# maxwellsh/DIGDriver

Measured on AMD Instinct MI355X. Metric: genomic elements tested/sec (whole node), whole-genome x 37 cohorts, higher is better.
Workload: dtype f64

## Files before the change

digdriver_amd/_lib.py:

```python
import ctypes
import os
import sys

import numpy as np

_HERE = os.path.dirname(os.path.abspath(__file__))
LIB_PATH = os.environ.get("DIG_HIP_LIB") or os.path.join(_HERE, "lib", "libdig_hip.so")

DIG_F32, DIG_F64, DIG_I16, DIG_BF16 = 0, 1, 2, 3
DIG_PIPE_CONTEXTS, DIG_PIPE_DOT, DIG_PIPE_STATISTICS, DIG_PIPE_WORKLIST_CLEAN, DIG_PIPE_COMPACT_L, DIG_PIPE_RECORDS = 1, 2, 4, 8, 16, 32
DIG_REC_DOUBLES, DIG_REC_MU, DIG_REC_SIGMA, DIG_REC_ROBS_FLAG = 10, 7, 8, 9
DIG_CNV_SCAN_CHUNK = 2048
GENE_CLASSES = ("SYN", "MIS", "NONS", "SPL", "TRUNC", "NONSYN")
GS_PLANES = tuple("EXP_" + c for c in GENE_CLASSES) + tuple("PVAL_%s_BURDEN" % c for c in GENE_CLASSES) + \
    tuple("PVAL_%s_BURDEN_SAMPLE" % c for c in GENE_CLASSES) + ("THETA_INDEL", "EXP_INDEL", "PVAL_INDEL_BURDEN", "PVAL_MUT_BURDEN")
SEL_PLANES = ("T_SYN", "MRFOLD") + tuple("EXP_%s_ML" % c for c in GENE_CLASSES) + \
    tuple("PVAL_%s_BURDEN_DNDS" % c for c in GENE_CLASSES) + tuple("PVAL_%s_SEL_NB" % c for c in ("SYN", "MIS", "TRUNC", "NONSYN")) + \
    tuple("PVAL_%s_SEL_PG" % c for c in ("SYN", "MIS", "NONS", "NONSYN")) + tuple("SEL_" + c for c in GENE_CLASSES) + \
    tuple("PVAL_%s_SEL" % c for c in GENE_CLASSES)
ES_PLANES = ("EXP_SNV", "PVAL_SNV_BURDEN", "PVAL_SAMPLE_BURDEN", "THETA_INDEL", "EXP_INDEL",
             "PVAL_INDEL_BURDEN", "PVAL_MUT_BURDEN")


class DigHipError(RuntimeError):
    pass


_lib = None
TORCH_FREE = False
_loaded_without_torch = False


def _need_torch():
# ... 11 lines not shown
    "dig_nb_exact_host": [_vp, _vp, _vp, _vp, _i64, _int],
    "dig_nb_greater": [_vp, _vp, _vp, _vp, _i64, _vp],
    "dig_nb_greater_host": [_vp, _vp, _vp, _vp, _i64, _int],
    "dig_nb_midp_twosided": [_vp, _vp, _vp, _vp, _i64, _vp],
    "dig_nb_midp_twosided_host": [_vp, _vp, _vp, _vp, _i64, _int],
    "dig_fisher": [_vp, _vp, _vp, _i64, _vp],
    "dig_fisher_host": [_vp, _vp, _vp, _i64, _int],
    "dig_normal_params_to_gamma": [_vp, _vp, _vp, _vp, _i64, _vp],
    "dig_normal_params_to_gamma_host": [_vp, _vp, _vp, _vp, _i64, _int],
    "dig_element_stats": [_vp, _vp, _vp, _vp, _vp, _vp, _int, _vp, _vp, _vp, _vp, _vp, _vp, _i64, _i64, _vp, _i64, _vp],
    "dig_element_stats_host": [_vp, _vp, _vp, _vp, _vp, _vp, _int, _vp, _vp, _vp, _vp, _vp, _vp, _i64, _i64, _int],
    "dig_accumulate_elements": [_vp] * 8 + [_int] + [_vp] * 11 + [_i64, _i64, _i64, _vp, _i64, _vp],
    "dig_accumulate_elements_host": [_vp] * 8 + [_int] + [_vp] * 11 + [_i64, _i64, _i64, _int],
    "dig_scale_suffstats": [_vp, _vp, _i64, _i64, _vp, _vp, _i64, _vp],
    "dig_scale_suffstats_host": [_vp, _vp, _i64, _i64, _vp, _int],
    "dig_scale_factors": [_vp, _int, _i64, _vp, _vp, _vp],
    "dig_scale_suffstats_chunked": [_vp, _vp, _i64, _vp, _int, _vp, _vp, _i64, _vp],
    "dig_scale_factors_chunked": [_vp, _int, _vp, _int, _i64, _vp, _vp, _vp, _vp],
    "dig_scale_factors_local": [_vp, _vp, _i64, _i64, _vp, _vp, _vp, _vp, _vp, _vp, _i64, _vp],
    "dig_element_pipeline": [_vp] * 25 + [_i64, _i64, _i64, _vp, _int, _vp, _i64, _vp],
    "dig_bin_records_pack": [_vp, _vp, _vp, _vp, _i64, _i64, _vp, _i64, _vp],
    "dig_element_records_unpack": [_vp, _i64, _i64, _vp, _vp, _vp, _vp, _vp, _int, _vp],
    "dig_element_pipeline_prepare": [_vp, _i64, _i64, _vp, _i64, _vp, _vp],
    "dig_element_pipeline_host": [_vp] * 25 + [_i64, _i64, _i64, _int],
    "dig_gene_stats": [_vp, _vp, _vp, _vp, _vp, _int, _vp, _int, _vp, _vp, _vp, _vp, _int, _vp, _i64, _i64, _vp],
    "dig_gene_stats_host": [_vp, _vp, _vp, _vp, _vp, _int, _vp, _int, _vp, _vp, _vp, _vp, _int, _vp, _i64, _i64, _int],
    "dig_gene_selection": [_vp, _vp, _vp, _int, _vp, _vp, _i64, _i64, _vp],
    "dig_gene_selection_host": [_vp, _vp, _vp, _int, _vp, _vp, _i64, _i64, _int],
    "dig_gene_row_keys": [_vp] * 5 + [_i64] * 4 + [_vp, _vp, _vp],
    "dig_gene_row_keys_host": [_vp] * 5 + [_i64] * 4 + [_vp, _vp, _int],
    "dig_gene_counts": [_vp, _i64, _vp, _i64, ctypes.c_double, ctypes.c_double, _i64, _i64, _i64] + [_vp] * 7,
    "dig_gene_counts_host": [_vp, _i64, _vp, _i64, ctypes.c_double, ctypes.c_double, _i64, _i64, _i64] + [_vp] * 5 + [_int],
    "dig_panel_row_keys": [_vp] * 7 + [_i64] * 5 + [_vp, _vp, _vp],
    "dig_panel_row_keys_host": [_vp] * 7 + [_i64] * 5 + [_vp, _vp, _int],
    "dig_panel_counts": [_vp, _i64, _vp, _vp] + [_i64] * 4 + [_vp] * 4,
    "dig_panel_counts_host": [_vp, _i64, _vp, _vp] + [_i64] * 4 + [_vp] * 3 + [_int],
    "dig_window_pair_keys": [_vp, _vp, _i64, _vp, _i64, _vp, _vp, _vp] + [_i64] * 4 + [_vp, _vp],
    "dig_window_pair_keys_host": [_vp, _vp, _i64, _vp, _i64, _vp, _vp, _vp] + [_i64] * 4 + [_vp, _int],
    "dig_window_sample_hits": [_vp] + [_i64] * 4 + [_vp, _vp],
    "dig_window_sample_hits_host": [_vp] + [_i64] * 4 + [_vp, _int],
    "dig_window_objectives": [_vp, _i64, _vp, _vp] + [_i64] * 4 + [_vp, _vp, _vp],
    "dig_window_objectives_host": [_vp, _i64, _vp, _vp] + [_i64] * 4 + [_vp, _int],
    "dig_cnv_segment_deltas": [_vp, _vp, _vp, _i64, _i64, _i64] + [_vp] * 6 + [_i64, _i64, _vp, _vp],
    "dig_cnv_segment_deltas_host": [_vp, _vp, _vp, _i64, _i64, _i64] + [_vp] * 6 + [_i64, _i64, _vp, _int],
    "dig_cnv_window_means": [_vp, _i64, _i64, _i64, _vp, _vp, _vp],
    "dig_cnv_window_means_host": [_vp, _i64, _i64, _i64, _vp, _int],
# ... 248 lines not shown
```

digdriver_amd/csrc/dig_accumulate.hip:

```cpp
#include <algorithm>
#include <type_traits>
#include <vector>

#include "dig_common.hpp"
#include "dig_math.hpp"

namespace dig {

constexpr int kAccLdsBudget = 160 * 1024 - 1024;

struct AccArgs {
    const double *bin_mu, *bin_std;
    const int32_t* bin_y;
    const uint8_t* bin_flag;
    const int32_t* bin_ctx;
    const int64_t* ov_ptr;
    const int32_t* ov_idx;
    const int32_t* L;
    const uint8_t* strand_minus;
    const int32_t* gene_length;
    const double* d_pr;
    double *MU, *SIGMA;
    int32_t *R_OBS, *FLAG;
    double* P;
// ... 494 lines not shown
            }
        }
        tile = tile_next;
    }
}

constexpr int kCtxWaves = 12;
constexpr int kCtxSteps = 16;

__global__ __launch_bounds__(256) void compact_L_kernel(const int32_t* __restrict__ L, int64_t n64, int32_t* __restrict__ Lc,
                                                        int* __restrict__ mismatch)
{
    const int64_t stride = (int64_t)gridDim.x * 256;
    int bad = 0;
    for (int64_t g = (int64_t)blockIdx.x * 256 + threadIdx.x; g < n64; g += stride) {
        const int32_t* p = L + 3 * g;
        const int a = p[0], b = p[1], c = p[2];
        Lc[g] = a;
        bad |= (a != b) | (a != c);
    }
    if (__any(bad) && (threadIdx.x & 63) == 0) atomicOr(mismatch, 1);
}

template <int NT, int NQ>
__global__ __launch_bounds__(kCtxWaves * 64) __attribute__((amdgpu_waves_per_eu(3, 3), amdgpu_num_vgpr(80))) void acc_dot_ctx_kernel(
    const int32_t* __restrict__ bin_ctx, const int64_t* __restrict__ ov_ptr, const int32_t* __restrict__ ov_idx,
    const uint8_t* __restrict__ strand_minus, const int32_t* __restrict__ Lc, const double* __restrict__ d_pr,
    const int32_t* __restrict__ gene_length, double* __restrict__ P, int32_t* __restrict__ R_SIZE,
    int32_t* __restrict__ ELT_SIZE, double* __restrict__ P_INDEL, int64_t E, int C, int c0, int write_sizes,
    unsigned* __restrict__ zero_dwords, int n_zero)
{
    constexpr int SL = NT + (NQ > 0 ? 1 : 0);
    constexpr int NTA = NT > 0 ? NT : 1, NQA = NQ > 0 ? NQ : 1;
    __shared__ double tab[kCtxSteps * SL * 64];

    if (zero_dwords && blockIdx.x == 0 && (int)threadIdx.x < n_zero) zero_dwords[threadIdx.x] = 0u;
    if (threadIdx.x < kChunkCohorts) g_cohort_bad[threadIdx.x] = 0u;
    __syncthreads();

    const int lane = threadIdx.x & 63, wave = __builtin_amdgcn_readfirstlane((int)(threadIdx.x >> 6));
    const int i = lane & 15, kq = lane >> 4;
    const int toff = 4 * kq + (lane & 3);
    const int64_t n_tiles = (E + 15) >> 4;
    const int nx = (gridDim.x & 7u) == 0u ? 8 : 1;
    const int xcd = blockIdx.x % nx, slot_b = blockIdx.x / nx, nslots = gridDim.x / nx;
    const int64_t per_x = (n_tiles + nx - 1) / nx;
    const int64_t t_begin = (int64_t)xcd * per_x;
    const int64_t t_end = t_begin + per_x < n_tiles ? t_begin + per_x : n_tiles;
    const int64_t stride = (int64_t)nslots * kCtxWaves;
    int64_t tile = t_begin + (int64_t)wave * nslots + slot_b;

    const int4* ctx4 = reinterpret_cast<const int4*>(bin_ctx);
    const int4* L4 = reinterpret_cast<const int4*>(Lc);
    const int64_t nnz = ov_ptr[E];
    const int32_t* oi_base = nnz > 0 ? ov_idx : reinterpret_cast<const int32_t*>(ov_ptr);
    const int64_t oi_last = nnz > 0 ? nnz - 1 : 0;

    struct Bounds { int64_t q0; int cm; };
    struct Idx { int i0, i1; };
    struct Rows { int4 a[4], b[4], l[4]; };
    auto first_row = [&](int64_t tile_) { return min(tile_, n_tiles - 1) * 16; };
    auto row_off = [&](int64_t row0) { return (unsigned)min(i, (int)min(E - 1 - row0, (int64_t)15)); };
    auto load_bounds = [&](int64_t tile_) {
        Bounds r;
        const int64_t row0 = first_row(tile_);
        const unsigned ro = row_off(row0);
        const int64_t* op = ov_ptr + row0;
        r.q0 = op[ro];
        const int cnt = (int)(op[ro + 1] - r.q0);
        r.cm = max(cnt, 0) | ((strand_minus + row0)[ro] ? (int)0x80000000u : 0);
        return r;
    };
    auto load_idx = [&](const Bounds& b) {
        Idx x;
        x.i0 = oi_base[min(b.q0, oi_last)];
        x.i1 = oi_base[min(b.q0 + 1, oi_last)];
        return x;
    };
    auto load_rows = [&](int64_t tile_, const Bounds& b, const Idx& x) {
        Rows r;
        const int kk = b.cm < 0 ? 3 - kq : kq;
        const int4* r0 = ctx4 + (int64_t)x.i0 * 16 + kk;
        const int4* r1 = ctx4 + (int64_t)x.i1 * 16 + kk;
        const int64_t row0 = first_row(tile_);
        const int4* rl = L4 + row0 * 16;
        const unsigned lo = row_off(row0) * 16u + (unsigned)kq;
#pragma unroll
        for (int t = 0; t < 4; ++t) r.a[t] = r0[4 * t];
#pragma unroll
        for (int t = 0; t < 4; ++t) r.b[t] = r1[4 * t];
#pragma unroll
        for (int t = 0; t < 4; ++t) r.l[t] = rl[lo + 4u * t];
        return r;
    };

    Bounds b_c = load_bounds(tile), b_n = load_bounds(tile + stride);
    Idx x_c = load_idx(b_c);

    {
        constexpr int kTotal = kCtxSteps * SL * 64;
        constexpr int kPer = (kTotal + kCtxWaves * 64 - 1) / (kCtxWaves * 64);
        double d0[kPer], d1[kPer], d2[kPer];
#pragma unroll
        for (int j = 0; j < kPer; ++j) {
            const int idx = threadIdx.x + j * kCtxWaves * 64;
            const int lane_ = idx & 63, slot = (idx >> 6) % SL, step = idx / (SL * 64);
            const bool tail = NQ > 0 && slot == NT;
            const int kappa = 16 * (step >> 2) + 4 * (tail ? (lane_ >> 2) & 3 : lane_ >> 4) + (step & 3);
            const int c = c0 + slot * 16 + (tail ? 4 * (lane_ >> 4) + (lane_ & 3) : lane_ & 15);
            d0[j] = d1[j] = d2[j] = 0.0;
            if (idx < kTotal && c < C && (!tail || (lane_ >> 4) < NQ)) {
                const double* d = d_pr + (int64_t)c * 192 + 3 * kappa;
                d0[j] = d[0];
// ... 2 lines not shown
                if (!(d0[j] > 0.0 && d1[j] > 0.0 && d2[j] > 0.0)) atomicOr(&g_cohort_bad[c - c0], 1u);
            }
        }
#pragma unroll
        for (int j = 0; j < kPer; ++j) {
            const int idx = threadIdx.x + j * kCtxWaves * 64;
            if (idx < kTotal) tab[idx] = (d0[j] + d1[j]) + d2[j];
        }
    }
    Rows r_c = load_rows(tile, b_c, x_c);
    __syncthreads();
    if (tile >= t_end) return;

    while (tile < t_end) {
        int opaque_zero;
        asm volatile("s_mov_b32 %0, 0" : "=s"(opaque_zero));
        const double* tabw = tab + opaque_zero;
        const int64_t e0 = tile * 16;
        const Bounds b_nn = load_bounds(tile + 2 * stride);
        const Idx x_n = load_idx(b_n);
        const int cnt = b_c.cm & 0x7fffffff;
        const bool minus = b_c.cm < 0;
        int rcv[4][4], lv[4][4];
        {
            const int m0 = cnt > 0 ? -1 : 0, m1 = cnt > 1 ? -1 : 0;
#pragma unroll
            for (int t = 0; t < 4; ++t) {
                rcv[t][0] = (r_c.a[t].x & m0) + (r_c.b[t].x & m1);
                rcv[t][1] = (r_c.a[t].y & m0) + (r_c.b[t].y & m1);
                rcv[t][2] = (r_c.a[t].z & m0) + (r_c.b[t].z & m1);
                rcv[t][3] = (r_c.a[t].w & m0) + (r_c.b[t].w & m1);
                lv[t][0] = r_c.l[t].x; lv[t][1] = r_c.l[t].y; lv[t][2] = r_c.l[t].z; lv[t][3] = r_c.l[t].w;
            }
        }
        if (__any(cnt > 2)) {
            const int kk = minus ? 3 - kq : kq;
            for (int j = 2; j < cnt; ++j) {
                const int4* r = ctx4 + (int64_t)ov_idx[b_c.q0 + j] * 16 + kk;
#pragma unroll
                for (int t = 0; t < 4; ++t) {
                    const int4 v = r[4 * t];
                    rcv[t][0] += v.x; rcv[t][1] += v.y; rcv[t][2] += v.z; rcv[t][3] += v.w;
                }
            }
        }
        int lzero = 0;
        {
            int rsum = 0, lsum = 0;
#pragma unroll
            for (int t = 0; t < 4; ++t) {
#pragma unroll
                for (int u = 0; u < 4; ++u) {
                    rsum += rcv[t][u];
                    lsum += lv[t][u];
                    lzero |= lv[t][u] == 0;
                }
            }
            if (write_sizes) {
// ... 2 lines not shown
                lsum += __shfl_xor(lsum, 16, 64);
                lsum += __shfl_xor(lsum, 32, 64);
                const unsigned io = (unsigned)(i + opaque_zero);
                if (kq == 0 && e0 + i < E) {
                    (R_SIZE + e0)[io] = rsum;
                    (ELT_SIZE + e0)[io] = lsum;
                    const double numer = gene_length ? (double)(gene_length + e0)[io] : (double)lsum;
                    (P_INDEL + e0)[io] = numer / (double)rsum;
                }
            }
        }
        double4_t den[NTA], num[NTA];
        double denq[NQA], numq[NQA];
#pragma unroll
        for (int nt = 0; nt < NTA; ++nt) den[nt] = num[nt] = double4_t{0.0, 0.0, 0.0, 0.0};
#pragma unroll
        for (int q = 0; q < NQA; ++q) denq[q] = numq[q] = 0.0;
        auto steps = [&](auto T0) {
            constexpr int t0 = decltype(T0)::value;
#pragma unroll
            for (int t = t0; t < t0 + 2; ++t) {
#pragma unroll
                for (int u = 0; u < 4; ++u) {
                    const int vr = minus ? rcv[3 - u][3 - t] : rcv[t][u];
                    const double Ar = (double)vr, Al = (double)lv[t][u];
                    const double* b = tabw + ((4 * t + u) * SL) * 64 + lane;
#pragma unroll
                    for (int nt = 0; nt < NT; ++nt) {
                        const double bv = b[nt * 64];
                        den[nt] = __builtin_amdgcn_mfma_f64_16x16x4f64(Ar, bv, den[nt], 0, 0, 0);
                        num[nt] = __builtin_amdgcn_mfma_f64_16x16x4f64(Al, bv, num[nt], 0, 0, 0);
                    }
                    if constexpr (NQ > 0) {
                        const double* bq = tabw + ((4 * t + u) * SL + NT) * 64 + toff;
#pragma unroll
                        for (int q = 0; q < NQ; ++q) {
                            const double bv = bq[q * 16];
                            denq[q] = __builtin_amdgcn_mfma_f64_4x4x4f64(Ar, bv, denq[q], 0, 0, 0);
                            numq[q] = __builtin_amdgcn_mfma_f64_4x4x4f64(Al, bv, numq[q], 0, 0, 0);
                        }
                    }
                }
            }
        };
        steps(std::integral_constant<int, 0>{});
        r_c = load_rows(tile + stride, b_n, x_n);
        steps(std::integral_constant<int, 2>{});
// ... 112 lines not shown
            int rc = (n_class == 1) ? launch_acc_v1<1>(a, s) : launch_acc_v1<4>(a, s);
            if (rc) return rc;
        }
        return DIG_OK;
    }
    DIG_REQUIRE(((uintptr_t)workspace & 255u) == 0, "workspace 256-byte aligned");
    const AccWorkspace w = acc_workspace_layout(workspace, E, C);
    DIG_REQUIRE(workspace_bytes >= w.bytes, "workspace smaller than dig_accumulate_workspace(E, C)");
    if (parts & 1) {
        const int grid = grid_for(do_rates ? E * C : E * 16, kRegionBlock, 8);
        hipLaunchKernelGGL(acc_region_kernel, dim3(grid), dim3(kRegionBlock), 0, s, bin_mu, bin_std, bin_y, bin_flag,
                           bin_ctx, ov_ptr, ov_idx, strand_minus, MU, SIGMA, R_OBS, FLAG, R_SIZE, w.rcp, E, C,
                           make_fastdiv(C), (int)(C >= 2), d_pr, w.tab, w.n48, do_rates, zero_dwords, n_zero);
        DIG_HIP_TRY(hipGetLastError());
    }
    if (!(parts & 2)) return DIG_OK;
    return (n_class == 1) ? launch_dot_mfma<1>(w, L, R_SIZE, gene_length, P, ELT_SIZE, P_INDEL, E, C, s, d_pr)
                          : launch_dot_mfma<4>(w, L, R_SIZE, gene_length, P, ELT_SIZE, P_INDEL, E, C, s, d_pr);
}

int accumulate_compact_launch(const int32_t* bin_ctx, const int64_t* ov_ptr, const int32_t* ov_idx, const uint8_t* strand_minus,
                              const int32_t* Lc, const int32_t* gene_length, const double* d_pr, double* P, int32_t* R_SIZE,
                              int32_t* ELT_SIZE, double* P_INDEL, int64_t E, int64_t C, void* stream, unsigned* zero_dwords,
                              int n_zero)
{
    if (E == 0 || C == 0) return DIG_OK;
    DIG_REQUIRE(bin_ctx && ov_ptr && ov_idx && strand_minus && Lc && d_pr, "non-null inputs");
    DIG_REQUIRE(P && R_SIZE && ELT_SIZE && P_INDEL, "non-null outputs");
    const int64_t n_tiles = (E + 15) / 16;
    int grid = (int)std::max<int64_t>(1, std::min<int64_t>(cu_count(), (n_tiles + kCtxWaves - 1) / kCtxWaves));
    if (grid >= 8) grid &= ~7;
    const int n48 = (int)((C + kMfmaChunk - 1) / kMfmaChunk);
    for (int ch = 0; ch < n48; ++ch) {
        const ChunkCut cut = chunk_cut((int)C, ch);
        const int rc = dispatch_cut(cut, [&](auto nt, auto nq) -> int {
            auto kern = acc_dot_ctx_kernel<nt.value, nq.value>;
            DIG_LAUNCH_STAGE(DIG_PIPE_DOT, kern, dim3(grid), dim3(kCtxWaves * 64), 0, (hipStream_t)stream, bin_ctx, ov_ptr, ov_idx, strand_minus,
                               Lc, d_pr, gene_length, P, R_SIZE, ELT_SIZE, P_INDEL, E, (int)C, ch * kMfmaChunk, (int)(ch == 0),
                               ch == 0 ? zero_dwords : nullptr, n_zero);
            DIG_HIP_TRY(hipGetLastError());
            return DIG_OK;
        });
        if (rc) return rc;
    }
    return DIG_OK;
}

int compact_L_launch(const int32_t* L, int64_t E, int32_t* Lc, int* mismatch, void* stream)
{
    DIG_HIP_TRY(hipMemsetAsync(mismatch, 0, sizeof(int), (hipStream_t)stream));
    if (E == 0) return DIG_OK;
    hipLaunchKernelGGL(compact_L_kernel, dim3(grid_for(E * 64, 256)), dim3(256), 0, (hipStream_t)stream, L, E * 64, Lc, mismatch);
    DIG_HIP_TRY(hipGetLastError());
    return DIG_OK;
}

}

extern "C" {

int dig_accumulate_elements(const double* bin_mu, const double* bin_std, const int32_t* bin_y, const uint8_t* bin_flag,
                            const int32_t* bin_ctx, const int64_t* ov_ptr, const int32_t* ov_idx, const int32_t* L,
                            int n_class, const uint8_t* strand_minus, const int32_t* gene_length, const double* d_pr,
                            double* MU, double* SIGMA, int32_t* R_OBS, int32_t* FLAG, double* P, int32_t* R_SIZE,
                            int32_t* ELT_SIZE, double* P_INDEL, int64_t N, int64_t E, int64_t C, void* workspace,
                            int64_t workspace_bytes, void* stream)
{
// ... 57 lines not shown
```

digdriver_amd/csrc/dig_pipeline.hip:

```cpp
#include <algorithm>
#include <vector>

#include "dig_common.hpp"

namespace dig {

struct FusedRates {
    const double *bin_mu, *bin_std;
    const int32_t* bin_y;
    const uint8_t* bin_flag;
    const int64_t* ov_ptr;
    const int32_t* ov_idx;
    double *mu_w, *sigma_w;
    int32_t *r_obs, *flag;
    int small_index;
    const double2* bin_pack;
    const int32_t* bin_yf;
    int records;
};

int accumulate_launch(const double* bin_mu, const double* bin_std, const int32_t* bin_y, const uint8_t* bin_flag,
                      const int32_t* bin_ctx, const int64_t* ov_ptr, const int32_t* ov_idx, const int32_t* L, int n_class,
                      const uint8_t* strand_minus, const int32_t* gene_length, const double* d_pr, double* MU,
                      double* SIGMA, int32_t* R_OBS, int32_t* FLAG, double* P, int32_t* R_SIZE, int32_t* ELT_SIZE,
                      double* P_INDEL, int64_t N, int64_t E, int64_t C, void* workspace, int64_t workspace_bytes,
                      void* stream, int do_rates, unsigned* zero_dwords, int n_zero, int parts);
int element_stats_launch(const double* mu, const double* sigma, const double* mu_indel, const double* sigma_indel,
                         const double* pi_sum, const double* pi_indel, int pi_indel_per_cohort, const int32_t* obs_snv,
                         const int32_t* obs_samples, const int32_t* obs_indel, const double* cj, const double* cj_indel,
                         double* out, int64_t E, int64_t C, void* workspace, int64_t workspace_bytes, void* stream,
                         const FusedRates* fused, int worklist_already_zero);
int accumulate_compact_launch(const int32_t* bin_ctx, const int64_t* ov_ptr, const int32_t* ov_idx, const uint8_t* strand_minus,
                              const int32_t* Lc, const int32_t* gene_length, const double* d_pr, double* P, int32_t* R_SIZE,
                              int32_t* ELT_SIZE, double* P_INDEL, int64_t E, int64_t C, void* stream, unsigned* zero_dwords,
                              int n_zero);
int compact_L_launch(const int32_t* L, int64_t E, int32_t* Lc, int* mismatch, void* stream);

struct PipeLayout {
    int64_t acc_bytes, stats_off, stats_bytes, lc_off, flag_off, bytes;
};
static PipeLayout pipe_layout(int64_t E, int64_t C, int64_t acc, int64_t stats)
{
    auto up = [](int64_t v) { return (v + 255) / 256 * 256; };
    PipeLayout p{};
    p.acc_bytes = up(acc);
    p.stats_off = p.acc_bytes;
    p.stats_bytes = stats;
    p.lc_off = up(p.stats_off + stats);
    p.flag_off = up(p.lc_off + E * 64 * (int64_t)sizeof(int32_t));
    p.bytes = p.flag_off + 256;
    return p;
}

__global__ __launch_bounds__(256) void pack_bins_kernel(const double* __restrict__ mu, const double* __restrict__ sd,
                                                        const int32_t* __restrict__ y, const uint8_t* __restrict__ fl, int64_t n,
                                                        double2* __restrict__ pack, int32_t* __restrict__ yf, int* __restrict__ bad)
{
#pragma clang fp contract(off)
// ... 63 lines not shown

int dig_element_pipeline_prepare(const int32_t* L, int64_t E, int64_t C, void* workspace, int64_t workspace_bytes,
                                 int* compact_ok, void* stream)
{
    DIG_REQUIRE(E >= 0 && C >= 0 && compact_ok, "E, C >= 0, compact_ok non-null");
    *compact_ok = 0;
    if (E == 0 || C == 0) return DIG_OK;
    DIG_REQUIRE(L, "L non-null");
    const int64_t need = dig_element_pipeline_workspace(E, C);
    DIG_REQUIRE(workspace && need > 0 && workspace_bytes >= need,
                "workspace of at least dig_element_pipeline_workspace(E, C) bytes (E * C must stay below 2^32 - 1)");
    DIG_REQUIRE(((uintptr_t)workspace & 255u) == 0, "workspace 256-byte aligned");
    const PipeLayout lay = pipe_layout(E, C, dig_accumulate_workspace(E, C), dig_element_stats_workspace(E, C));
    int* flag = (int*)((char*)workspace + lay.flag_off);
    int rc = compact_L_launch(L, E, (int32_t*)((char*)workspace + lay.lc_off), flag, stream);
    if (rc) return rc;
    int bad = 1;
    DIG_HIP_TRY(hipMemcpyAsync(&bad, flag, sizeof(int), hipMemcpyDeviceToHost, (hipStream_t)stream));
    DIG_HIP_TRY(hipStreamSynchronize((hipStream_t)stream));
    *compact_ok = bad ? 0 : 1;
    return DIG_OK;
}

int64_t dig_element_records_bytes(int64_t E, int64_t C)
{
    if (E <= 0 || C <= 0) return 0;
    return (E * C + 63) / 64 * 64 * DIG_REC_DOUBLES * (int64_t)sizeof(double);
}

int dig_element_records_unpack(const double* records, int64_t E, int64_t C, double* out7, double* MU, double* SIGMA,
                               int32_t* R_OBS, int32_t* FLAG, int cohort_major, void* stream)
{
    DIG_REQUIRE(E >= 0 && C >= 0, "E, C >= 0");
    if (E == 0 || C == 0) return DIG_OK;
    DIG_REQUIRE(records, "records non-null");
    hipLaunchKernelGGL(records_unpack_kernel, dim3(grid_for(E * C, 256)), dim3(256), 0, (hipStream_t)stream, records, E, C, out7, MU,
                       SIGMA, R_OBS, FLAG, cohort_major);
    DIG_HIP_TRY(hipGetLastError());
    return DIG_OK;
}

int64_t dig_bin_records_bytes(int64_t N, int64_t C)
{
    if (N <= 0 || C <= 0) return 0;
    return bin_records_layout(N, C).bytes;
}
// ... 35 lines not shown
                         int32_t* R_SIZE, int32_t* ELT_SIZE, double* P_INDEL, double* out, int64_t N, int64_t E, int64_t C,
                         const void* bin_records, int stages, void* workspace, int64_t workspace_bytes, void* stream)
{
    const int rc = element_pipeline_run(bin_mu, bin_std, bin_y, bin_flag, bin_ctx, ov_ptr, ov_idx, L, strand_minus, gene_length, d_pr,
                                        obs_snv, obs_samples, obs_indel, cj, cj_indel, MU, SIGMA, R_OBS, FLAG, P, R_SIZE, ELT_SIZE,
                                        P_INDEL, out, N, E, C, bin_records, stages, workspace, workspace_bytes, stream);
    dig::disarm_stage_timers();
    return rc;
}

}

static int element_pipeline_run(const double* bin_mu, const double* bin_std, const int32_t* bin_y, const uint8_t* bin_flag,
                         const int32_t* bin_ctx, const int64_t* ov_ptr, const int32_t* ov_idx, const int32_t* L,
                         const uint8_t* strand_minus, const int32_t* gene_length, const double* d_pr,
                         const int32_t* obs_snv, const int32_t* obs_samples, const int32_t* obs_indel, const double* cj,
                         const double* cj_indel, double* MU, double* SIGMA, int32_t* R_OBS, int32_t* FLAG, double* P,
                         int32_t* R_SIZE, int32_t* ELT_SIZE, double* P_INDEL, double* out, int64_t N, int64_t E, int64_t C,
                         const void* bin_records, int stages, void* workspace, int64_t workspace_bytes, void* stream)
{
    const int worklist_clean = (stages & DIG_PIPE_WORKLIST_CLEAN) != 0;
    const int compact = (stages & DIG_PIPE_COMPACT_L) != 0 && N >= 1;
    const int records = (stages & DIG_PIPE_RECORDS) != 0;
    stages &= ~(DIG_PIPE_WORKLIST_CLEAN | DIG_PIPE_COMPACT_L | DIG_PIPE_RECORDS);
    DIG_REQUIRE(stages >= 1 && stages <= 7, "stages: bit mask of DIG_PIPE_CONTEXTS, DIG_PIPE_DOT, DIG_PIPE_STATISTICS");
    DIG_REQUIRE(N >= 0 && E >= 0 && C >= 0, "N, E, C >= 0");
    if (E == 0 || C == 0) return DIG_OK;
    DIG_REQUIRE(obs_snv && obs_samples && obs_indel && cj && cj_indel && out, "non-null statistics arguments");
    const int64_t need = dig_element_pipeline_workspace(E, C);
    DIG_REQUIRE(workspace && need > 0 && workspace_bytes >= need,
                "workspace of at least dig_element_pipeline_workspace(E, C) bytes (E * C must stay below 2^32 - 1)");
    DIG_REQUIRE(((uintptr_t)workspace & 255u) == 0, "workspace 256-byte aligned");
    const PipeLayout lay = pipe_layout(E, C, dig_accumulate_workspace(E, C), dig_element_stats_workspace(E, C));
    const int64_t acc_bytes = lay.acc_bytes;
    unsigned* wl = (unsigned*)((char*)workspace + acc_bytes);
    if (compact) {
        if (stages & DIG_PIPE_DOT) {
            DIG_REQUIRE(bin_ctx && ov_ptr && ov_idx && strand_minus && d_pr && P && R_SIZE && ELT_SIZE && P_INDEL,
                        "non-null accumulation arguments");
            int rc = accumulate_compact_launch(bin_ctx, ov_ptr, ov_idx, strand_minus, (const int32_t*)((char*)workspace + lay.lc_off),
                                               gene_length, d_pr, P, R_SIZE, ELT_SIZE, P_INDEL, E, C, stream, wl, 64);
            if (rc) return rc;
        }
    } else if (stages & 3) {
        int rc = accumulate_launch(bin_mu, bin_std, bin_y, bin_flag, bin_ctx, ov_ptr, ov_idx, L, 1, strand_minus, gene_length,
                                   d_pr, MU, SIGMA, R_OBS, FLAG, P, R_SIZE, ELT_SIZE, P_INDEL, N, E, C, workspace, acc_bytes,
                                   stream, 0, wl, 64, stages & 3);
        if (rc) return rc;
    }
    if (!(stages & 4)) return DIG_OK;
    const int small_index = N < ((int64_t)1 << 24) && C < ((int64_t)1 << 24) && N * C < ((int64_t)1 << 32);
    FusedRates f{bin_mu, bin_std, bin_y, bin_flag, ov_ptr, ov_idx, MU, SIGMA, R_OBS, FLAG, small_index, nullptr, nullptr, records};
    if (records) {
        DIG_REQUIRE(bin_records, "DIG_PIPE_RECORDS needs bin_records (dig_bin_records_pack)");
        DIG_REQUIRE(((uintptr_t)out & 255u) == 0, "record-major `out` 256-byte aligned");
    }
    if (bin_records) {
        const BinRecords lay_r = bin_records_layout(N, C);
        f.bin_pack = (const double2*)bin_records;
        f.bin_yf = (const int32_t*)((const char*)bin_records + lay_r.yf_off);
    }
    return element_stats_launch(MU, SIGMA, nullptr, nullptr, P, P_INDEL, 0, obs_snv, obs_samples, obs_indel, cj, cj_indel,
                                out, E, C, (char*)workspace + acc_bytes, lay.stats_bytes, stream, &f,
                                (compact ? (stages & DIG_PIPE_DOT) != 0 : (stages & 1) != 0) || worklist_clean);
// ... 2 lines not shown
```

digdriver_amd/engine.py:

```python
import contextlib

import numpy as np

from . import _lib
from ._marshal import backend_of, backend_on, device_backend, is_cuda

ES_PLANES = _lib.ES_PLANES
GS_PLANES = _lib.GS_PLANES
SEL_PLANES = _lib.SEL_PLANES


def _t(x, dtype, device):
    return device_backend(device).arr(x, dtype)


_WS_CACHE = {}


def _workspace(kind, E, C, dev, private=False):
    import torch
    need = _lib.workspace_bytes(kind, E, C)
    if need <= 0:
        return None, 0
    if private:
# ... 455 lines not shown
        ov_idx = be.arr([0], "i32")
    return [bin_mu, be.arr(bin_std, "f64", (N, C)), be.arr(bin_y, "i32", (N, C)), be.arr(bin_flag, "u8", (N, C)),
            be.arr(bin_ctx, "i32", (N, 64)), ov_ptr, ov_idx, L, be.arr(strand_minus, "u8"), be.arr(gene_length, "i32"),
            be.arr(d_pr, "f64", (C, 192))], (N, E, C, n_class)


def accumulate_elements(bin_mu, bin_std, bin_y, bin_flag, bin_ctx, ov_ptr, ov_idx, L, strand_minus, d_pr,
                        gene_length=None, device=0, out=None, use_workspace=True):
    be = backend_of(bin_mu, device=device)
    tabs, (N, E, C, n_class) = _bin_tables(be, bin_mu, bin_std, bin_y, bin_flag, bin_ctx, ov_ptr, ov_idx, L, strand_minus,
                                           gene_length, d_pr)
    o = out if out is not None else _accumulate_outputs(be, E, C, n_class)
    p = [be.ptr(x) for x in tabs]
    be.call("dig_accumulate_elements", *p[:8], n_class, *p[8:], *[be.ptr(o[k]) for k in _ACC_OUTPUTS], N, E, C,
            workspace=_shared_workspace(be, "accumulate", E, C, use_workspace))
    return o


def element_pipeline(bin_mu, bin_std, bin_y, bin_flag, bin_ctx, ov_ptr, ov_idx, L, strand_minus, d_pr, obs_snv,
                     obs_samples, obs_indel, cj, cj_indel, gene_length=None, out_acc=None, out_stats=None, stages=7, compact=False):
    if compact:
        plan = PipelinePlan(bin_mu, bin_std, bin_y, bin_flag, bin_ctx, ov_ptr, ov_idx, L, strand_minus, d_pr, obs_snv, obs_samples,
                            obs_indel, out_acc=out_acc, out_stats=out_stats, gene_length=gene_length, compact=compact,
                            pack_bins=False)
        return plan.run(_t(cj, "f64", plan.dev), _t(cj_indel, "f64", plan.dev), stages=stages)
    be = device_backend(bin_mu.device)
    tabs, (N, E, C, n_class) = _bin_tables(be, bin_mu, bin_std, bin_y, bin_flag, bin_ctx, ov_ptr, ov_idx, L, strand_minus,
                                           gene_length, d_pr)
    assert n_class == 1
    obs = [be.arr(x, "i32") for x in (obs_snv, obs_samples, obs_indel)]
    assert all(x.shape == (E, C) for x in obs)
    cj, cj_indel = be.arr(cj, "f64"), be.arr(cj_indel, "f64")
    o = out_acc if out_acc is not None else _accumulate_outputs(be, E, C, 1)
    st = out_stats if out_stats is not None else be.empty((len(ES_PLANES), E, C), "f64")
    ws = _shared_workspace(be, "pipeline", E, C)
    if ws[0] is None:
        raise _lib.DigHipError("dig_element_pipeline: problem too large for the fused path (E * C >= 2^32 - 1)")
    p = be.ptr
    be.call("dig_element_pipeline", *[p(x) for x in tabs], *[p(x) for x in obs], p(cj), p(cj_indel), *[p(o[k]) for k in _ACC_OUTPUTS],
            p(st), N, E, C, None, int(stages), workspace=ws)
    return o, st


_RECORDS_FASTER = {}


def records_form_is_faster(plane_plan, record_plan, cj, cj_indel, rounds=2, warm=8, launches=25):
# ... 6 lines not shown
        for name, pl in (("planes", plane_plan), ("records", record_plan)):
            best = float("inf")
            for _ in range(rounds):
                ea, eb = torch.cuda.Event(enable_timing=True), torch.cuda.Event(enable_timing=True)
                for _w in range(warm):
                    pl.run(cj, cj_indel)
                ea.record()
                for _r in range(launches):
                    pl.run(cj, cj_indel)
                eb.record()
                eb.synchronize()
                best = min(best, ea.elapsed_time(eb) / launches * 1e3)
            us[name] = best
    _RECORDS_FASTER[key] = (us["records"] < us["planes"] - 1.5, us)
    return _RECORDS_FASTER[key]


class PipelinePlan:

    _ws_owner = {}

    def __init__(self, bin_mu, bin_std, bin_y, bin_flag, bin_ctx, ov_ptr, ov_idx, L, strand_minus, d_pr, obs_snv,
                 obs_samples, obs_indel, out_acc=None, out_stats=None, gene_length=None, compact="auto", workspace=None,
                 pack_bins=True, records_out=False):
        import ctypes
        import torch
        dev = bin_mu.device
        be = device_backend(dev)
        tabs, (self.N, self.E, self.C, n_class) = _bin_tables(be, bin_mu, bin_std, bin_y, bin_flag, bin_ctx, ov_ptr, ov_idx, L,
                                                              strand_minus, gene_length, d_pr)
        assert n_class == 1
        L = tabs[7]
        self.keep = tabs + [be.arr(x, "i32") for x in (obs_snv, obs_samples, obs_indel)]
        assert all(x.shape == (self.E, self.C) for x in self.keep[11:14])
        self.dev = dev
        self.acc = out_acc if out_acc is not None else _accumulate_outputs(be, self.E, self.C, 1)
        self.stats = out_stats if out_stats is not None else be.empty((len(ES_PLANES), self.E, self.C), "f64")
        if workspace is not None:
            self.ws, self.wsb = workspace, _lib.workspace_bytes("pipeline", self.E, self.C)
            assert workspace.numel() >= self.wsb and workspace.data_ptr() % 256 == 0
            import weakref
            owner = PipelinePlan._ws_owner.get(workspace.data_ptr())
            if owner is not None and owner[0]() is not None and owner[0]() is not self and owner[1] != (L.data_ptr(), tuple(L.shape)):
                raise ValueError("this workspace buffer already belongs to a live PipelinePlan over ANOTHER element set (a compact "
                                 "plan keeps its copy of L in it): give every plan its own workspace")
            PipelinePlan._ws_owner[workspace.data_ptr()] = (weakref.ref(self), (L.data_ptr(), tuple(L.shape)))
        else:
# ... 12 lines not shown
            self.records = torch.empty(nb, dtype=torch.uint8, device=dev)
            self.repack_bins()
        self.records_out = bool(records_out)
        self.out_records = None
        if self.records_out:
            if self.records is None:
                raise ValueError("records_out needs the packed bin records (pack_bins)")
            nrec = (self.E * self.C + 63) // 64 * 64
            self.out_records = torch.empty((nrec // 64, _lib.DIG_REC_DOUBLES // 2, 64, 2), dtype=torch.float64, device=dev)
            assert self.out_records.data_ptr() % 256 == 0
        self._tail = [p(o["MU"]), p(o["SIGMA"]), p(o["R_OBS"]), p(o["FLAG"]), p(o["P"]), p(o["R_SIZE"]), p(o["ELT_SIZE"]),
                      p(o["P_INDEL"]), p(self.out_records if self.records_out else self.stats), self.N, self.E, self.C,
                      p(self.records)]
        self._ws = p(self.ws)
        self._fn = getattr(_lib.load(), "dig_element_pipeline")
        self.compact = False
        if compact and self.N >= 1:
            ok = ctypes.c_int(0)
            with torch.cuda.device(dev):
                _lib.call("dig_element_pipeline_prepare", p(L), self.E, self.C, self._ws, self.wsb, ctypes.byref(ok),
                          _lib.stream_ptr())
            self.compact = bool(ok.value)
        self._flags = (_lib.DIG_PIPE_COMPACT_L if self.compact else 0) | (_lib.DIG_PIPE_RECORDS if self.records_out else 0)

    def unpack(self, cohort_major=False, stream=None, stats=None, rates=None):
        import torch
        assert self.records_out
        p = _lib.dev_ptr
        o = self.acc
        with torch.cuda.device(self.dev):
            if cohort_major:
                assert stats is not None and tuple(stats.shape) == (len(ES_PLANES), self.C, self.E)
                r = rates or {}
                assert all(tuple(v.shape) == (self.C, self.E) and v.is_contiguous() for v in r.values())
                assert all(r[k].dtype == (torch.float64 if k in ("MU", "SIGMA") else torch.int32) for k in r)
                _lib.call("dig_element_records_unpack", p(self.out_records), self.E, self.C, p(stats), p(r.get("MU")), p(r.get("SIGMA")),
                          p(r.get("R_OBS")), p(r.get("FLAG")), 1, _lib.stream_ptr(stream))
                return stats
            st = self.stats if stats is None else stats
            _lib.call("dig_element_records_unpack", p(self.out_records), self.E, self.C, p(st), p(o["MU"]), p(o["SIGMA"]),
                      p(o["R_OBS"]), p(o["FLAG"]), 0, _lib.stream_ptr(stream))
        return o, st

    def repack_bins(self):
        import torch
        if self.records is None:
            return
        k = self.keep
        with torch.cuda.device(self.dev):
            _lib.call("dig_bin_records_pack", _lib.dev_ptr(k[0]), _lib.dev_ptr(k[1]), _lib.dev_ptr(k[2]), _lib.dev_ptr(k[3]),
                      self.N, self.C, _lib.dev_ptr(self.records), self.records.numel(), _lib.stream_ptr())

    def run(self, cj, cj_indel, stages=7, stream=None):
        rc = self._fn(*self._head, _lib.dev_ptr(cj), _lib.dev_ptr(cj_indel), *self._tail, int(stages) | self._flags, self._ws,
                      self.wsb, _lib.stream_ptr(stream))
        _lib.check("dig_element_pipeline", rc)
        return self.acc, self.stats


class PlanRing:

    def __init__(self, plans, streams=None):
        import torch
        self.plans = list(plans)
        assert self.plans, "at least one plan"
        dev = self.plans[0].dev
        self.streams = list(streams) if streams is not None else [torch.cuda.Stream(device=dev) for _ in self.plans]
        assert len(self.streams) == len(self.plans)

    def run(self, k, cj, cj_indel):
        j = k % len(self.plans)
        return self.plans[j].run(cj, cj_indel, stream=self.streams[j])

    def synchronize(self):
# ... 822 lines not shown
```

include/dig_hip.h:

```cpp
#ifndef DIG_HIP_H
#define DIG_HIP_H

#include <stdint.h>

#ifdef __cplusplus
extern "C" {
#endif

#define DIG_OK 0
#define DIG_EINVAL (-1)
#define DIG_EHIP (-2)
#define DIG_ENODEV (-3)

#define DIG_ABI_VERSION 12

#define DIG_F32 0
#define DIG_F64 1
#define DIG_I16 2
#define DIG_BF16 3

#define DIG_ES_EXP_SNV 0
#define DIG_ES_PVAL_SNV_BURDEN 1
#define DIG_ES_PVAL_SAMPLE_BURDEN 2
#define DIG_ES_THETA_INDEL 3
// ... 40 lines not shown

int64_t dig_accumulate_workspace(int64_t E, int64_t C);
int dig_accumulate_elements(const double *bin_mu, const double *bin_std, const int32_t *bin_y,
                            const uint8_t *bin_flag, const int32_t *bin_ctx, const int64_t *ov_ptr,
                            const int32_t *ov_idx, const int32_t *L, int n_class, const uint8_t *strand_minus,
                            const int32_t *gene_length, const double *d_pr, double *MU, double *SIGMA,
                            int32_t *R_OBS, int32_t *FLAG, double *P, int32_t *R_SIZE, int32_t *ELT_SIZE,
                            double *P_INDEL, int64_t N, int64_t E, int64_t C, void *workspace,
                            int64_t workspace_bytes, void *stream);
int dig_accumulate_elements_host(const double *bin_mu, const double *bin_std, const int32_t *bin_y,
                                 const uint8_t *bin_flag, const int32_t *bin_ctx, const int64_t *ov_ptr,
                                 const int32_t *ov_idx, const int32_t *L, int n_class, const uint8_t *strand_minus,
                                 const int32_t *gene_length, const double *d_pr, double *MU, double *SIGMA,
                                 int32_t *R_OBS, int32_t *FLAG, double *P, int32_t *R_SIZE, int32_t *ELT_SIZE,
                                 double *P_INDEL, int64_t N, int64_t E, int64_t C, int device);

#define DIG_PIPE_CONTEXTS 1
#define DIG_PIPE_DOT 2
#define DIG_PIPE_ACCUMULATE 3
#define DIG_PIPE_STATISTICS 4
#define DIG_PIPE_ALL 7
#define DIG_PIPE_WORKLIST_CLEAN 8
#define DIG_PIPE_COMPACT_L 16
#define DIG_PIPE_RECORDS 32
#define DIG_REC_DOUBLES 10
#define DIG_REC_MU 7
#define DIG_REC_SIGMA 8
#define DIG_REC_ROBS_FLAG 9
int64_t dig_element_records_bytes(int64_t E, int64_t C);
int dig_element_records_unpack(const double *records, int64_t E, int64_t C, double *out7, double *MU, double *SIGMA,
                               int32_t *R_OBS, int32_t *FLAG, int cohort_major, void *stream);
int64_t dig_element_pipeline_workspace(int64_t E, int64_t C);
int dig_stage_timer_create(void **timer);
int dig_stage_timer_arm(void *timer, int stage);
int dig_stage_timer_read(void *timer, double *ms);
int dig_stage_timer_selftest(void *timer, void *stream);
int dig_stage_timer_destroy(void *timer);
int dig_element_pipeline_prepare(const int32_t *L, int64_t E, int64_t C, void *workspace, int64_t workspace_bytes,
                                 int *compact_ok, void *stream);
int dig_element_pipeline_host(const double *bin_mu, const double *bin_std, const int32_t *bin_y, const uint8_t *bin_flag,
                              const int32_t *bin_ctx, const int64_t *ov_ptr, const int32_t *ov_idx, const int32_t *L,
                              const uint8_t *strand_minus, const int32_t *gene_length, const double *d_pr,
                              const int32_t *obs_snv, const int32_t *obs_samples, const int32_t *obs_indel, const double *cj,
                              const double *cj_indel, double *MU, double *SIGMA, int32_t *R_OBS, int32_t *FLAG, double *P,
                              int32_t *R_SIZE, int32_t *ELT_SIZE, double *P_INDEL, double *out, int64_t N, int64_t E, int64_t C,
                              int device);
// ... 438 lines not shown
```

Before: 26.49 billion.

## Precompute per-element summed context table and read it densely in dot kernel

Adds a kernel that sums each element's overlapping bin context rows and applies reverse-complement for minus-strand elements, writing a dense E×64 int table once per plan. A new PLANNED variant of the dot kernel reads this table row-contiguously, like L. This drops the per-tile ov_ptr/ov_idx gathers, the extra loop for elements with more than two bins, and the strand-dependent index swaps. The cost is an extra E×64 int32 buffer, built at plan construction and shared between plans with the same structure. If the bin contexts change, recontext() must be called.

```diff
diff --git a/digdriver_amd/_lib.py b/digdriver_amd/_lib.py
--- a/digdriver_amd/_lib.py
+++ b/digdriver_amd/_lib.py
@@ -9,6 +9,7 @@
 
 DIG_F32, DIG_F64, DIG_I16, DIG_BF16 = 0, 1, 2, 3
 DIG_PIPE_CONTEXTS, DIG_PIPE_DOT, DIG_PIPE_STATISTICS, DIG_PIPE_WORKLIST_CLEAN, DIG_PIPE_COMPACT_L, DIG_PIPE_RECORDS = 1, 2, 4, 8, 16, 32
+DIG_PIPE_ELEMENT_CTX = 64
 DIG_REC_DOUBLES, DIG_REC_MU, DIG_REC_SIGMA, DIG_REC_ROBS_FLAG = 10, 7, 8, 9
 DIG_CNV_SCAN_CHUNK = 2048
 GENE_CLASSES = ("SYN", "MIS", "NONS", "SPL", "TRUNC", "NONSYN")
@@ -66,6 +67,7 @@
     "dig_bin_records_pack": [_vp, _vp, _vp, _vp, _i64, _i64, _vp, _i64, _vp],
     "dig_element_records_unpack": [_vp, _i64, _i64, _vp, _vp, _vp, _vp, _vp, _int, _vp],
     "dig_element_pipeline_prepare": [_vp, _i64, _i64, _vp, _i64, _vp, _vp],
+    "dig_element_contexts_prepare": [_vp, _vp, _vp, _vp, _i64, _i64, _vp, _vp],
     "dig_element_pipeline_host": [_vp] * 25 + [_i64, _i64, _i64, _int],
     "dig_gene_stats": [_vp, _vp, _vp, _vp, _vp, _int, _vp, _int, _vp, _vp, _vp, _vp, _int, _vp, _i64, _i64, _vp],
     "dig_gene_stats_host": [_vp, _vp, _vp, _vp, _vp, _int, _vp, _int, _vp, _vp, _vp, _vp, _int, _vp, _i64, _i64, _int],
diff --git a/digdriver_amd/csrc/dig_accumulate.hip b/digdriver_amd/csrc/dig_accumulate.hip
--- a/digdriver_amd/csrc/dig_accumulate.hip
+++ b/digdriver_amd/csrc/dig_accumulate.hip
@@ -540,7 +540,34 @@
     if (__any(bad) && (threadIdx.x & 63) == 0) atomicOr(mismatch, 1);
 }
 
-template <int NT, int NQ>
+__global__ __launch_bounds__(256) void element_contexts_kernel(const int32_t* __restrict__ bin_ctx, const int64_t* __restrict__ ov_ptr,
+                                                               const int32_t* __restrict__ ov_idx, const uint8_t* __restrict__ strand_minus,
+                                                               int64_t E, int32_t* __restrict__ elt_ctx)
+{
+    const int l16 = threadIdx.x & 15;
+    const int4* ctx4 = reinterpret_cast<const int4*>(bin_ctx);
+    const int64_t stride = ((int64_t)gridDim.x * 256) >> 4;
+    for (int64_t e = ((int64_t)blockIdx.x * 256 + threadIdx.x) >> 4; e < E; e += stride) {
+        const int64_t q0 = ov_ptr[e], q1 = ov_ptr[e + 1];
+        int4 acc = make_int4(0, 0, 0, 0);
+        for (int64_t q = q0; q < q1; ++q) {
+            const int4 v = ctx4[(int64_t)ov_idx[q] * 16 + l16];
+            acc.x += v.x; acc.y += v.y; acc.z += v.z; acc.w += v.w;
+        }
+        if (!strand_minus[e]) {
+            reinterpret_cast<int4*>(elt_ctx)[e * 16 + l16] = acc;
+        } else {
+            int32_t* row = elt_ctx + e * 64;
+            const int c0 = 4 * l16;
+            row[revcomp_ctx(c0 + 0)] = acc.x;
+            row[revcomp_ctx(c0 + 1)] = acc.y;
+            row[revcomp_ctx(c0 + 2)] = acc.z;
+            row[revcomp_ctx(c0 + 3)] = acc.w;
+        }
+    }
+}
+
+template <int NT, int NQ, bool PLANNED>
 __global__ __launch_bounds__(kCtxWaves * 64) __attribute__((amdgpu_waves_per_eu(3, 3), amdgpu_num_vgpr(80))) void acc_dot_ctx_kernel(
     const int32_t* __restrict__ bin_ctx, const int64_t* __restrict__ ov_ptr, const int32_t* __restrict__ ov_idx,
     const uint8_t* __restrict__ strand_minus, const int32_t* __restrict__ Lc, const double* __restrict__ d_pr,
@@ -570,17 +597,18 @@
 
     const int4* ctx4 = reinterpret_cast<const int4*>(bin_ctx);
     const int4* L4 = reinterpret_cast<const int4*>(Lc);
-    const int64_t nnz = ov_ptr[E];
+    const int64_t nnz = PLANNED ? 0 : ov_ptr[E];
     const int32_t* oi_base = nnz > 0 ? ov_idx : reinterpret_cast<const int32_t*>(ov_ptr);
     const int64_t oi_last = nnz > 0 ? nnz - 1 : 0;
 
     struct Bounds { int64_t q0; int cm; };
     struct Idx { int i0, i1; };
-    struct Rows { int4 a[4], b[4], l[4]; };
+    struct Rows { int4 a[4], b[PLANNED ? 1 : 4], l[4]; };
     auto first_row = [&](int64_t tile_) { return min(tile_, n_tiles - 1) * 16; };
     auto row_off = [&](int64_t row0) { return (unsigned)min(i, (int)min(E - 1 - row0, (int64_t)15)); };
     auto load_bounds = [&](int64_t tile_) {
-        Bounds r;
+        Bounds r{0, 0};
+        if constexpr (PLANNED) return r;
         const int64_t row0 = first_row(tile_);
         const unsigned ro = row_off(row0);
         const int64_t* op = ov_ptr + row0;
@@ -590,23 +618,31 @@
         return r;
     };
     auto load_idx = [&](const Bounds& b) {
-        Idx x;
+        Idx x{0, 0};
+        if constexpr (PLANNED) return x;
         x.i0 = oi_base[min(b.q0, oi_last)];
         x.i1 = oi_base[min(b.q0 + 1, oi_last)];
         return x;
     };
     auto load_rows = [&](int64_t tile_, const Bounds& b, const Idx& x) {
         Rows r;
-        const int kk = b.cm < 0 ? 3 - kq : kq;
-        const int4* r0 = ctx4 + (int64_t)x.i0 * 16 + kk;
-        const int4* r1 = ctx4 + (int64_t)x.i1 * 16 + kk;
         const int64_t row0 = first_row(tile_);
         const int4* rl = L4 + row0 * 16;
         const unsigned lo = row_off(row0) * 16u + (unsigned)kq;
-#pragma unroll
-        for (int t = 0; t < 4; ++t) r.a[t] = r0[4 * t];
-#pragma unroll
-        for (int t = 0; t < 4; ++t) r.b[t] = r1[4 * t];
+        if constexpr (PLANNED) {
+            const int4* rr = ctx4 + row0 * 16;
+            r.b[0] = make_int4(0, 0, 0, 0);
+#pragma unroll
+            for (int t = 0; t < 4; ++t) r.a[t] = rr[lo + 4u * t];
+        } else {
+            const int kk = b.cm < 0 ? 3 - kq : kq;
+            const int4* r0 = ctx4 + (int64_t)x.i0 * 16 + kk;
+            const int4* r1 = ctx4 + (int64_t)x.i1 * 16 + kk;
+#pragma unroll
+            for (int t = 0; t < 4; ++t) r.a[t] = r0[4 * t];
+#pragma unroll
+            for (int t = 0; t < 4; ++t) r.b[t] = r1[4 * t];
+        }
 #pragma unroll
         for (int t = 0; t < 4; ++t) r.l[t] = rl[lo + 4u * t];
         return r;
@@ -655,7 +691,13 @@
         const int cnt = b_c.cm & 0x7fffffff;
         const bool minus = b_c.cm < 0;
         int rcv[4][4], lv[4][4];
-        {
+        if constexpr (PLANNED) {
+#pragma unroll
+            for (int t = 0; t < 4; ++t) {
+                rcv[t][0] = r_c.a[t].x; rcv[t][1] = r_c.a[t].y; rcv[t][2] = r_c.a[t].z; rcv[t][3] = r_c.a[t].w;
+                lv[t][0] = r_c.l[t].x; lv[t][1] = r_c.l[t].y; lv[t][2] = r_c.l[t].z; lv[t][3] = r_c.l[t].w;
+            }
+        } else {
             const int m0 = cnt > 0 ? -1 : 0, m1 = cnt > 1 ? -1 : 0;
 #pragma unroll
             for (int t = 0; t < 4; ++t) {
@@ -666,7 +708,7 @@
                 lv[t][0] = r_c.l[t].x; lv[t][1] = r_c.l[t].y; lv[t][2] = r_c.l[t].z; lv[t][3] = r_c.l[t].w;
             }
         }
-        if (__any(cnt > 2)) {
+        if (!PLANNED && __any(cnt > 2)) {
             const int kk = minus ? 3 - kq : kq;
             for (int j = 2; j < cnt; ++j) {
                 const int4* r = ctx4 + (int64_t)ov_idx[b_c.q0 + j] * 16 + kk;
@@ -715,7 +757,7 @@
             for (int t = t0; t < t0 + 2; ++t) {
 #pragma unroll
                 for (int u = 0; u < 4; ++u) {
-                    const int vr = minus ? rcv[3 - u][3 - t] : rcv[t][u];
+                    const int vr = !PLANNED && minus ? rcv[3 - u][3 - t] : rcv[t][u];
                     const double Ar = (double)vr, Al = (double)lv[t][u];
                     const double* b = tabw + ((4 * t + u) * SL) * 64 + lane;
 #pragma unroll
@@ -874,10 +916,11 @@
 int accumulate_compact_launch(const int32_t* bin_ctx, const int64_t* ov_ptr, const int32_t* ov_idx, const uint8_t* strand_minus,
                               const int32_t* Lc, const int32_t* gene_length, const double* d_pr, double* P, int32_t* R_SIZE,
                               int32_t* ELT_SIZE, double* P_INDEL, int64_t E, int64_t C, void* stream, unsigned* zero_dwords,
-                              int n_zero)
+                              int n_zero, int planned)
 {
     if (E == 0 || C == 0) return DIG_OK;
-    DIG_REQUIRE(bin_ctx && ov_ptr && ov_idx && strand_minus && Lc && d_pr, "non-null inputs");
+    DIG_REQUIRE(bin_ctx && Lc && d_pr && (planned || (ov_ptr && ov_idx && strand_minus)), "non-null inputs");
+    DIG_REQUIRE(!planned || ((uintptr_t)bin_ctx & 255u) == 0, "element context table (DIG_PIPE_ELEMENT_CTX) 256-byte aligned");
     DIG_REQUIRE(P && R_SIZE && ELT_SIZE && P_INDEL, "non-null outputs");
     const int64_t n_tiles = (E + 15) / 16;
     int grid = (int)std::max<int64_t>(1, std::min<int64_t>(cu_count(), (n_tiles + kCtxWaves - 1) / kCtxWaves));
@@ -886,7 +929,7 @@
     for (int ch = 0; ch < n48; ++ch) {
         const ChunkCut cut = chunk_cut((int)C, ch);
         const int rc = dispatch_cut(cut, [&](auto nt, auto nq) -> int {
-            auto kern = acc_dot_ctx_kernel<nt.value, nq.value>;
+            auto kern = planned ? acc_dot_ctx_kernel<nt.value, nq.value, true> : acc_dot_ctx_kernel<nt.value, nq.value, false>;
             DIG_LAUNCH_STAGE(DIG_PIPE_DOT, kern, dim3(grid), dim3(kCtxWaves * 64), 0, (hipStream_t)stream, bin_ctx, ov_ptr, ov_idx, strand_minus,
                                Lc, d_pr, gene_length, P, R_SIZE, ELT_SIZE, P_INDEL, E, (int)C, ch * kMfmaChunk, (int)(ch == 0),
                                ch == 0 ? zero_dwords : nullptr, n_zero);
@@ -895,6 +938,15 @@
         });
         if (rc) return rc;
     }
+    return DIG_OK;
+}
+
+int element_contexts_launch(const int32_t* bin_ctx, const int64_t* ov_ptr, const int32_t* ov_idx, const uint8_t* strand_minus, int64_t E,
+                            int32_t* elt_ctx, void* stream)
+{
+    hipLaunchKernelGGL(element_contexts_kernel, dim3(grid_for(E * 16, 256)), dim3(256), 0, (hipStream_t)stream, bin_ctx, ov_ptr, ov_idx,
+                       strand_minus, E, elt_ctx);
+    DIG_HIP_TRY(hipGetLastError());
     return DIG_OK;
 }
 
diff --git a/digdriver_amd/csrc/dig_pipeline.hip b/digdriver_amd/csrc/dig_pipeline.hip
--- a/digdriver_amd/csrc/dig_pipeline.hip
+++ b/digdriver_amd/csrc/dig_pipeline.hip
@@ -33,7 +33,9 @@
 int accumulate_compact_launch(const int32_t* bin_ctx, const int64_t* ov_ptr, const int32_t* ov_idx, const uint8_t* strand_minus,
                               const int32_t* Lc, const int32_t* gene_length, const double* d_pr, double* P, int32_t* R_SIZE,
                               int32_t* ELT_SIZE, double* P_INDEL, int64_t E, int64_t C, void* stream, unsigned* zero_dwords,
-                              int n_zero);
+                              int n_zero, int planned);
+int element_contexts_launch(const int32_t* bin_ctx, const int64_t* ov_ptr, const int32_t* ov_idx, const uint8_t* strand_minus, int64_t E,
+                            int32_t* elt_ctx, void* stream);
 int compact_L_launch(const int32_t* L, int64_t E, int32_t* Lc, int* mismatch, void* stream);
 
 struct PipeLayout {
@@ -143,6 +145,17 @@
     return DIG_OK;
 }
 
+int dig_element_contexts_prepare(const int32_t* bin_ctx, const int64_t* ov_ptr, const int32_t* ov_idx, const uint8_t* strand_minus,
+                                 int64_t N, int64_t E, int32_t* elt_ctx, void* stream)
+{
+    DIG_REQUIRE(N >= 0 && E >= 0, "N, E >= 0");
+    if (E == 0) return DIG_OK;
+    DIG_REQUIRE(ov_ptr && strand_minus && elt_ctx, "ov_ptr, strand_minus, elt_ctx non-null");
+    DIG_REQUIRE(N == 0 || (bin_ctx && ov_idx), "bin_ctx, ov_idx non-null");
+    DIG_REQUIRE(((uintptr_t)elt_ctx & 255u) == 0, "elt_ctx 256-byte aligned");
+    return element_contexts_launch(bin_ctx, ov_ptr, ov_idx, strand_minus, E, elt_ctx, stream);
+}
+
 int64_t dig_element_records_bytes(int64_t E, int64_t C)
 {
     if (E <= 0 || C <= 0) return 0;
@@ -224,7 +237,11 @@
     const int worklist_clean = (stages & DIG_PIPE_WORKLIST_CLEAN) != 0;
     const int compact = (stages & DIG_PIPE_COMPACT_L) != 0 && N >= 1;
     const int records = (stages & DIG_PIPE_RECORDS) != 0;
-    stages &= ~(DIG_PIPE_WORKLIST_CLEAN | DIG_PIPE_COMPACT_L | DIG_PIPE_RECORDS);
+    const int planned = (stages & DIG_PIPE_ELEMENT_CTX) != 0;
+    DIG_REQUIRE(!planned || (stages & DIG_PIPE_COMPACT_L), "DIG_PIPE_ELEMENT_CTX is valid only together with DIG_PIPE_COMPACT_L");
+    DIG_REQUIRE(!planned || N >= 1, "DIG_PIPE_ELEMENT_CTX needs N >= 1 (the compact form)");
+    DIG_REQUIRE(!planned || ((uintptr_t)bin_ctx & 255u) == 0, "element context table (DIG_PIPE_ELEMENT_CTX) 256-byte aligned");
+    stages &= ~(DIG_PIPE_WORKLIST_CLEAN | DIG_PIPE_COMPACT_L | DIG_PIPE_RECORDS | DIG_PIPE_ELEMENT_CTX);
     DIG_REQUIRE(stages >= 1 && stages <= 7, "stages: bit mask of DIG_PIPE_CONTEXTS, DIG_PIPE_DOT, DIG_PIPE_STATISTICS");
     DIG_REQUIRE(N >= 0 && E >= 0 && C >= 0, "N, E, C >= 0");
     if (E == 0 || C == 0) return DIG_OK;
@@ -241,7 +258,7 @@
             DIG_REQUIRE(bin_ctx && ov_ptr && ov_idx && strand_minus && d_pr && P && R_SIZE && ELT_SIZE && P_INDEL,
                         "non-null accumulation arguments");
             int rc = accumulate_compact_launch(bin_ctx, ov_ptr, ov_idx, strand_minus, (const int32_t*)((char*)workspace + lay.lc_off),
-                                               gene_length, d_pr, P, R_SIZE, ELT_SIZE, P_INDEL, E, C, stream, wl, 64);
+                                               gene_length, d_pr, P, R_SIZE, ELT_SIZE, P_INDEL, E, C, stream, wl, 64, planned);
             if (rc) return rc;
         }
     } else if (stages & 3) {
diff --git a/digdriver_amd/engine.py b/digdriver_amd/engine.py
--- a/digdriver_amd/engine.py
+++ b/digdriver_amd/engine.py
@@ -501,7 +501,7 @@
     if compact:
         plan = PipelinePlan(bin_mu, bin_std, bin_y, bin_flag, bin_ctx, ov_ptr, ov_idx, L, strand_minus, d_pr, obs_snv, obs_samples,
                             obs_indel, out_acc=out_acc, out_stats=out_stats, gene_length=gene_length, compact=compact,
-                            pack_bins=False)
+                            pack_bins=False, element_contexts=False)
         return plan.run(_t(cj, "f64", plan.dev), _t(cj_indel, "f64", plan.dev), stages=stages)
     be = device_backend(bin_mu.device)
     tabs, (N, E, C, n_class) = _bin_tables(be, bin_mu, bin_std, bin_y, bin_flag, bin_ctx, ov_ptr, ov_idx, L, strand_minus,
@@ -554,7 +554,7 @@
 
     def __init__(self, bin_mu, bin_std, bin_y, bin_flag, bin_ctx, ov_ptr, ov_idx, L, strand_minus, d_pr, obs_snv,
                  obs_samples, obs_indel, out_acc=None, out_stats=None, gene_length=None, compact="auto", workspace=None,
-                 pack_bins=True, records_out=False):
+                 pack_bins=True, records_out=False, element_contexts=True):
         import ctypes
         import torch
         dev = bin_mu.device
@@ -613,6 +613,19 @@
                           _lib.stream_ptr())
             self.compact = bool(ok.value)
         self._flags = (_lib.DIG_PIPE_COMPACT_L if self.compact else 0) | (_lib.DIG_PIPE_RECORDS if self.records_out else 0)
+        self.elt_ctx = None
+        if self.compact and element_contexts:
+            if isinstance(element_contexts, PipelinePlan):
+                other = element_contexts
+                assert other.elt_ctx is not None and (other.N, other.E) == (self.N, self.E)
+                assert all(other.keep[i].data_ptr() == self.keep[i].data_ptr() for i in (4, 5, 6, 8))
+                self.elt_ctx = other.elt_ctx
+            else:
+                self.elt_ctx = torch.empty((self.E, 64), dtype=torch.int32, device=dev)
+                assert self.elt_ctx.data_ptr() % 256 == 0
+                self.recontext()
+            self._head[4] = p(self.elt_ctx)
+            self._flags |= _lib.DIG_PIPE_ELEMENT_CTX
 
     def unpack(self, cohort_major=False, stream=None, stats=None, rates=None):
         import torch
@@ -641,6 +654,15 @@
         with torch.cuda.device(self.dev):
             _lib.call("dig_bin_records_pack", _lib.dev_ptr(k[0]), _lib.dev_ptr(k[1]), _lib.dev_ptr(k[2]), _lib.dev_ptr(k[3]),
                       self.N, self.C, _lib.dev_ptr(self.records), self.records.numel(), _lib.stream_ptr())
+
+    def recontext(self):
+        import torch
+        if self.elt_ctx is None:
+            return
+        k = self.keep
+        with torch.cuda.device(self.dev):
+            _lib.call("dig_element_contexts_prepare", _lib.dev_ptr(k[4]), _lib.dev_ptr(k[5]), _lib.dev_ptr(k[6]), _lib.dev_ptr(k[8]),
+                      self.N, self.E, _lib.dev_ptr(self.elt_ctx), _lib.stream_ptr())
 
     def run(self, cj, cj_indel, stages=7, stream=None):
         rc = self._fn(*self._head, _lib.dev_ptr(cj), _lib.dev_ptr(cj_indel), *self._tail, int(stages) | self._flags, self._ws,
diff --git a/include/dig_hip.h b/include/dig_hip.h
--- a/include/dig_hip.h
+++ b/include/dig_hip.h
@@ -86,6 +86,9 @@
 #define DIG_PIPE_ALL 7
 #define DIG_PIPE_WORKLIST_CLEAN 8
 #define DIG_PIPE_COMPACT_L 16
+#define DIG_PIPE_ELEMENT_CTX 64
+int dig_element_contexts_prepare(const int32_t *bin_ctx, const int64_t *ov_ptr, const int32_t *ov_idx,
+                                 const uint8_t *strand_minus, int64_t N, int64_t E, int32_t *elt_ctx, void *stream);
 #define DIG_PIPE_RECORDS 32
 #define DIG_REC_DOUBLES 10
 #define DIG_REC_MU 7
```

Result: faster. 26.89 billion, median of 6 (+1.5%).
